# TingweiMeng/PDHG-optimal-control

Measured on AMD Instinct MI355X. Metric: PDHG iterations/sec and achieved HBM GB/s on nt×nx[×ny] grid, 1/2/4/8 MI355X, higher is better.
Workload: dtype f64

## Files before the change

### pdhg-optimal-control_amd/csrc/ctx_impl.hpp

```cpp
#pragma once

#include <hip/hip_runtime.h>

#include <algorithm>
#include <climits>
#include <cmath>
#include <cstring>
#include <map>
#include <memory>
#include <string>
#include <type_traits>
#include <utility>
#include <vector>

#include "kernels_1d.hpp"
#include "kernels_2d.hpp"
#include "kernels_2d_fast.hpp"
#include "kernels_dual_lds.hpp"
#include "kernels_dual_multi.hpp"
#include "kernels_common.hpp"
#include "kernels_xslab.hpp"
#include "kernels_xt_batch.hpp"
#include "kernels_xt_dma.hpp"
#include "kernels_thomas_chunk.hpp"
// ... 608 lines not shown
          default: return fail(PDHG_ERR_UNSUPPORTED, "no batched x kernel for nx=%d", p.nx);
        }
        if (pp.fast_xt_code == 2) switch (p.nx) {
          case 8192: return launch(k_precond_xt_ws_2d<4096, 1, true>, g, dim3(512), lds, p, twx);
          case 4096: return launch(k_precond_xt_ws_2d<4096, 1>, g, dim3(512), lds, p, twx);
          case 2048: return launch(k_precond_xt_ws_2d<2048, 2>, g, dim3(512), lds, p, twx);
          case 1024: return launch(k_precond_xt_ws_2d<1024, 4>, g, dim3(512), lds, p, twx);
          case 512: return launch(k_precond_xt_ws_2d<512, 8>, g, dim3(512), lds, p, twx);
          default: return fail(PDHG_ERR_UNSUPPORTED, "no fast x kernel for nx=%d", p.nx);
        }
        switch (p.nx) {
          case 4096: return launch(k_precond_xt_fast_2d<4096, 1, 512>, g, dim3(512), lds, p, twx);
          case 2048: return launch(k_precond_xt_fast_2d<2048, 2, 512>, g, dim3(512), lds, p, twx);
          case 1024: return launch(k_precond_xt_fast_2d<1024, 4, 512>, g, dim3(512), lds, p, twx);
          case 512: return launch(k_precond_xt_fast_2d<512, 8, 512>, g, dim3(512), lds, p, twx);
          default: return fail(PDHG_ERR_UNSUPPORTED, "no fast x kernel for nx=%d", p.nx);
        }
      }
    } else {
      if (pp.t1_xt64 && one_row) {
        const bool g16 = pp.t1_g16;
        const size_t lds = (size_t)((p.B / 2) * (p.nx + p.nx / 16) + (g16 ? 48 : twlds_size(p.nx))) * sizeof(C);
        switch (p.nx) {
          case 4096:
            if (g16) return launch(k_precond_x_t1_2d<4096, 1, 512, double, true>, g, dim3(512), lds, p, twx);
            return launch(k_precond_x_t1_2d<4096, 1, 512, double>, g, dim3(512), lds, p, twx);
          case 2048:
            if (g16) return launch(k_precond_x_t1_2d<2048, 1, 256, double, true>, g, dim3(256), lds, p, twx);
            return launch(k_precond_x_t1_2d<2048, 1, 256, double>, g, dim3(256), lds, p, twx);
          case 1024: return launch(k_precond_x_t1_2d<1024, 2, 512, double>, g, dim3(512), lds, p, twx);
          case 512: return launch(k_precond_x_t1_2d<512, 4, 512, double>, g, dim3(512), lds, p, twx);
          default: return fail(PDHG_ERR_UNSUPPORTED, "no fp64 one-row x kernel for nx=%d", p.nx);
        }
      }
      if (pp.f64_xt) {
        if (pp.half_real)
          return launch(k_precond_xt_f64_2d<4096, 512, true>, g, dim3(512),
                        (size_t)(Pad<4096>::LINE + TwLds<4096>::SIZE + 4096 + 128) * sizeof(C), p, twx);
        if (p.nx == 1024)
          return launch(k_precond_xt_f64_2d<1024, 256, false, true>, g, dim3(256),
                        (size_t)(Pad<1024>::LINE + TwLds<1024>::SIZE) * sizeof(C), p, twx);
        if (p.nx == 512)
          return launch(k_precond_xt_f64_2d<512, 128, false, true>, g, dim3(128),
                        (size_t)(Pad<512>::LINE + TwLds<512>::SIZE) * sizeof(C), p, twx);
        if (p.nx == 2048) {
          const size_t bpr = (size_t)(Pad<2048>::LINE + TwLds<2048>::SIZE) * sizeof(C);
          switch (pp.xt64_var) {
            case 1: return launch(k_precond_xt_f64_2d<2048, 256, false, false>, g, dim3(256), bpr + 2048 * sizeof(C), p, twx);
            case 2: return launch(k_precond_xt_f64_2d<2048, 256, false, true>, g, dim3(256), bpr, p, twx);
            case 3: return launch(k_precond_xt_f64_2d<2048, 1024, false, true>, g, dim3(1024), bpr, p, twx);
            default: return launch(k_precond_xt_f64_2d<2048, 512, false, true>, g, dim3(512), bpr, p, twx);
          }
        }
        if (pp.xt64_dma) {
          if (p.rspec) return launch(k_precond_xt_f64_2d<4096, 512, false, true, true, true>, g, dim3(512), 0, p, twx);
          return launch(k_precond_xt_f64_2d<4096, 512, false, true, false, true>, g, dim3(512), 0, p, twx);
        }
        if (pp.xt64_bpr) {
          const size_t ldsr = (size_t)(Pad<4096>::LINE + TwLds<4096>::SIZE) * sizeof(C);
          if (p.rspec) return launch(k_precond_xt_f64_2d<4096, 512, false, true, true>, g, dim3(512), ldsr, p, twx);
          return launch(k_precond_xt_f64_2d<4096, 512, false, true>, g, dim3(512), ldsr, p, twx);
        }
        const size_t lds = (size_t)(Pad<4096>::LINE + TwLds<4096>::SIZE + 4096) * sizeof(C);
        if (p.rspec)
          return launch(k_precond_xt_f64_2d<4096, 512, false, false, true>, g, dim3(512), lds, p, twx);
        return launch(k_precond_xt_f64_2d<4096, 512>, g, dim3(512), lds, p, twx);
      }
    }
    return with_xt_fft([&](auto f) {
      return launch(k_precond_xt_2d<R, decltype(f)>, g, dim3(pp.NT2), pp.lds_xt, p, f, twx);
    });
  }

  int launch_update_2d(const KP<R>& p, int& upd_rows) {
    ProfScope ps(this, "update");
    const dim3 gf(pp.g_fast_upd);
    upd_rows = pp.g_fast_upd;
    if constexpr (sizeof(R) == 8) {
      if (pp.res64) {
        if (pb.ny == 2048 && pp.upd_t1 > 0) {
          const size_t lds = pp.lds_res64 + (size_t)48 * sizeof(C);
          if (pp.upd_t1 == 2) return launch(k_invy_update_fast_2d<2048, 4, 256, 2, double, true>, gf, dim3(256), lds, p, twy);
          return launch(k_invy_update_fast_2d<2048, 4, 256, 4, double, true>, gf, dim3(256), lds, p, twy);
        }
        if (pb.ny == 4096) return launch(k_invy_update_fast_2d<4096, 4, 512, 4, double>, gf, dim3(512), pp.lds_upd64, p, twy);
        return launch(k_invy_update_fast_2d<2048, 4, 512, 4, double>, gf, dim3(512), pp.lds_upd64, p, twy);
      }
      if (pp.upd8192)
        return launch(k_invy_update_fast_2d<8192, 2, 512, 2, double>, gf, dim3(512),
                      (size_t)Pad<8192>::LINE * sizeof(C), p, twy);
    }
    if constexpr (kMixed) {
      if (pp.fast_rows)
        return with_fast_rows([&](auto Nc, auto RWc, auto NTc) {
          constexpr int N_ = decltype(Nc)::value, RW_ = decltype(RWc)::value, NT_ = decltype(NTc)::value;
          if constexpr (NT_ == 1024 && RW_ == 8) {
            if (pp.upd_threads == 512)
              return launch(k_invy_update_fast_mixed_2d<N_, RW_, 512, kMixedUpdPF>, gf, dim3(512), pp.lds_fast_tw, p,
                            twy, px);
          }
          return launch(k_invy_update_fast_mixed_2d<N_, RW_, NT_>, gf, dim3(NT_), pp.lds_fast_tw, p, twy, px);
        });
      upd_rows = pp.gx4 * pp.g4;
      return with_line_fft(pp.ply, [&](auto f) {
        using F = decltype(f);
        if (pp.nt_row <= 256)
          return launch(k_invy_update_mixed_2d<F, 256>, dim3(pp.gx4), dim3(pp.nt_row), pp.lds_res, p, f, twy, px);
        return launch(k_invy_update_mixed_2d<F, 1024>, dim3(pp.gx4), dim3(pp.nt_row), pp.lds_res, p, f, twy, px);
      });
    }
    if (pp.fast_rows)
      return with_fast_rows([&](auto Nc, auto RWc, auto NTc) {
        constexpr int N_ = decltype(Nc)::value, RW_ = decltype(RWc)::value, NT_ = decltype(NTc)::value;
        if constexpr (sizeof(R) == 4) {
          if constexpr (NT_ == 1024 && RW_ == 8) {
            if (pp.upd_threads == 512) switch (pp.upd_pf) {
              case 2: return launch(k_invy_update_fast_2d<N_, RW_, 512, 2>, gf, dim3(512), pp.lds_fast_tw, p, twy);
              case 3: return launch(k_invy_update_fast_2d<N_, RW_, 512, 3>, gf, dim3(512), pp.lds_fast_tw, p, twy);
              case 4: return launch(k_invy_update_fast_2d<N_, RW_, 512, 4>, gf, dim3(512), pp.lds_fast_tw, p, twy);
              default: return launch(k_invy_update_fast_2d<N_, RW_, 512, 1>, gf, dim3(512), pp.lds_fast_tw, p, twy);
            }
          }
          return launch(k_invy_update_fast_2d<N_, RW_, NT_>, gf, dim3(NT_), pp.lds_fast_tw, p, twy);
        }
        return (int)PDHG_OK;
      });
    upd_rows = pp.gx4 * pp.g4;
    return with_line_fft(pp.ply, [&](auto f) {
      using F = decltype(f);
      if (pp.nt_row <= 256)
        return launch(k_invy_update_2d<R, F, 256>, dim3(pp.gx4), dim3(pp.nt_row), pp.lds_res, p, f, twy);
      return launch(k_invy_update_2d<R, F, 1024>, dim3(pp.gx4), dim3(pp.nt_row), pp.lds_res, p, f, twy);
    });
  }

  int launch_primal(R tau, int stages = 7, int xt_phase = 0, double* sums_out = nullptr) {
    KP<R> p = kp;
    p.tau = tau;
    p.xt_phase = xt_phase;
    const int T = pb.T;
    int rc;
    if (pb.ndim == 2) {
      if ((stages & 1) && (rc = launch_residual(p, 0, T))) return rc;
      if ((stages & 2) && (rc = launch_precond(p))) return rc;
      if (!(stages & 4)) return PDHG_OK;
      const bool prim_merge = spec && pp.fin_merge && !pp.dual_multi && !sums_out;
      if (prim_merge) p.partials = prim_partials;
      int upd_rows = 0;
      if ((rc = launch_update_2d(p, upd_rows))) return rc;
      if (sums_out)
        return launch(k_reduce_vec, dim3(1), dim3(1024), 0, p.partials, upd_rows, 3, kp.j0 == 0 ? row0_sq : 0.0,
                      sums_out);
      if (prim_merge) {
        prim_merged_rows = upd_rows;
        return PDHG_OK;
      }
      return launch(k_finalize_primal, dim3(1), dim3(1024), 0, p.partials, upd_rows, 1, p.ctrl);
    }
    if constexpr (kMixed) return fail(PDHG_ERR_STATE, "mixed context is 2-D only");
    if (pp.fourstep) return launch_fourstep_1d(p);
    {
      ProfScope ps(this, "residual");
      rc = with_line_fft(pp.plx, [&](auto f) {
        using F = decltype(f);
        return with_egno<2>([&](auto eg) {
          return launch(k_res_fwdx_1d<R, decltype(eg)::value, F>, dim3(pp.gx1), dim3(pp.nt1d), pp.lds_res, p, f, twx);
// ... 1189 lines not shown
```

### pdhg-optimal-control_amd/csrc/kernels_2d_fast.hpp

```cpp
#pragma once
#include <type_traits>
#include "params.hpp"

namespace pdhg {

__device__ __forceinline__ float4 ld4(const float* p) { return *reinterpret_cast<const float4*>(p); }
__device__ __forceinline__ void st4(float* p, float4 v) { *reinterpret_cast<float4*>(p) = v; }
__device__ __forceinline__ float f4(const float4& v, int e) { return e == 0 ? v.x : e == 1 ? v.y : e == 2 ? v.z : v.w; }
__device__ __forceinline__ void f4set(float4& v, int e, float x) {
  if (e == 0) v.x = x; else if (e == 1) v.y = x; else if (e == 2) v.z = x; else v.w = x;
}
__device__ __forceinline__ float4 z4() { return make_float4(0.f, 0.f, 0.f, 0.f); }

struct dbl4 {
  double x, y, z, w;
};
template <typename R> struct V4s { using type = float4; };
template <> struct V4s<double> { using type = dbl4; };
template <typename R> using V4 = typename V4s<R>::type;
__device__ __forceinline__ dbl4 ld4(const double* p) {
  const double2 a = reinterpret_cast<const double2*>(p)[0], b = reinterpret_cast<const double2*>(p)[1];
  return dbl4{a.x, a.y, b.x, b.y};
}
__device__ __forceinline__ void st4(double* p, dbl4 v) {
// ... 643 lines not shown
      }
#pragma unroll
      for (int i = 0; i < BATCH; ++i) {
        const int t = tl + (i0 + i) * NT;
        const int b = t >> lCS4, part = t & (CS4 - 1);
        if (B == 2) {
          C* Al = A + part * Pad<N>::LINE;
          Al[pix(2 * b)] = cmk<C>(v[i].x, v[i].z);
          Al[pix(2 * b + 1)] = cmk<C>(v[i].y, v[i].w);
        } else {
#pragma unroll
          for (int e = 0; e < 4; ++e) {
            const int f = part * 4 + e;
            const int r = f >> lB, c = f & (B - 1);
            Af[((r >> 1) * Pad<N>::LINE + pix(b * B + c)) * 2 + (r & 1)] = f4(v[i], e);
          }
        }
      }
    }
    R* phi = p.phi + (size_t)(j + 1) * plane;
    R* pbar = p.phibar + (size_t)(j + 1) * plane;
    constexpr int NS = GPT * NL;
    V op[NS][2];
    auto ldstep = [&](int s) {
      const size_t idx = (size_t)(x0 + 2 * (s % NL)) * N + 4 * (tid + (s / NL) * NT);
      op[s][0] = ld4(phi + idx);
      op[s][1] = ld4(phi + idx + N);
    };
    ldstep(0);
    lds_sync();
    if (!(p.dbg & 64)) {
      if constexpr (TWL && G16) lds_fft_inplace_tl16<C, N, NL, NT, Pad<N>::LINE>(A, twl, twy);
      else if constexpr (TWL) lds_fft_inplace_tl<C, N, NL, NT, Pad<N>::LINE>(A, twl);
      else lds_fft_inplace<C, N, NL, NT>(A, twy);
    }
#pragma unroll
    for (int s = 1; s < PF && s < NS; ++s) ldstep(s);
#pragma unroll
    for (int gi = 0; gi < GPT; ++gi) {
      const int y = 4 * (tid + gi * NT);
#pragma unroll
      for (int l = 0; l < NL; ++l) {
        const int st = gi * NL + l;
        const V o4[2] = {op[st][0], op[st][1]};
        if (st + PF < NS) ldstep(st + PF);
        const C* Z = A + l * Pad<N>::LINE;
        V u[2];
#pragma unroll
        for (int e = 0; e < 4; ++e) {
          R a, b2;
          hartley_padded<C, R>(Z, N, y + e, a, b2);
          f4set(u[0], e, a);
          f4set(u[1], e, b2);
        }
#pragma unroll
        for (int h = 0; h < 2; ++h) {
          const int xr = x0 + 2 * l + h;
          if (xr < p.xl0 || xr >= p.xl1) continue;
          const size_t idx = (size_t)xr * N + y;
          V nw, pb;
          R fs[3] = {(R)0, (R)0, (R)0};
#pragma unroll
          for (int e = 0; e < 4; ++e) {
            const R o = f4(o4[h], e);
            const R n = o + scale * f4(u[h], e);
            f4set(nw, e, n);
            f4set(pb, e, (R)2 * n - o);
            const R d = n - o;
            fs[0] = fmar(d, d, fs[0]);
            fs[1] = fmar(o, o, fs[1]);
            fs[2] = fmar(n, n, fs[2]);
          }
#pragma unroll
          for (int i = 0; i < 3; ++i) s[i] += (double)fs[i];
          st4(phi + idx, nw);
          st4(pbar + idx, pb);
        }
      }
    }
    lds_sync();
  }
  block_reduce_store<3>(s, p.partials, blockIdx.x);
}
template <int N, int RW, int NT, int PF = 1>
__global__ void __launch_bounds__(NT) k_invy_update_fast_mixed_2d(KP<float> p, const float2* __restrict__ twy,
                                                                  PhiX<float, double> px) {
  invy_update_fast_body<N, RW, NT, PF, float, false, double>(p, px, twy);
}

}

namespace pdhg {

__device__ __forceinline__ float expm1_neg(float x) {
  const float p = x * (1.f + x * (0.5f + x * (1.f / 6 + x * (1.f / 24 + x * (1.f / 120 + x * (1.f / 720 + x * (1.f / 5040)))))));
  return x > -0.25f ? p : __expf(x) - 1.f;
}

__device__ __forceinline__ float2 expm1_neg2(float a, float b) {
  float ea = __expf(a) - 1.f, eb = __expf(b) - 1.f;
  const bool sa = a > -0.25f, sb = b > -0.25f;
  if (__ballot(sa || sb) != 0) {
    auto poly = [](float x) {
      return x * (1.f + x * (0.5f + x * (1.f / 6 + x * (1.f / 24 + x * (1.f / 120 + x * (1.f / 720 + x * (1.f / 5040)))))));
    };
    if (sa) ea = poly(a);
    if (sb) eb = poly(b);
  }
  return make_float2(ea, eb);
}

__device__ __forceinline__ float h_entry(float dd, int j0) {
  if (j0 == 0) return 1.f;
  const float dl = 0.5f * dd;
  const float th = fmaxf(log1pf(dl + sqrtf(dl * (dl + 2.f))), 1e-20f);
  return expm1f(-th) * (1.f + expf(-th * (float)(2 * j0 + 1))) / expm1f(-2.f * th * (float)(j0 + 1));
}
__device__ __forceinline__ double h_entry(double dd, int j0) {
  if (j0 == 0) return 1.0;
  const double dl = 0.5 * dd;
  const double th = fmax(log1p(dl + sqrt(dl * (dl + 2.0))), 1e-300);
  return expm1(-th) * (1.0 + exp(-th * (double)(2 * j0 + 1))) / expm1(-2.0 * th * (double)(j0 + 1));
}

template <int N, int NL, int NT>
__global__ void __launch_bounds__(NT) k_precond_xt_fast_2d(KP<float> p, const float2* __restrict__ twx) {
  using C = float2;
  constexpr int IT = N * NL / NT;
  constexpr int B = 2 * NL;
  constexpr int NI = N * NL;
  constexpr int LINE = Pad<N>::LINE;
  constexpr int lnl = (NL == 1) ? 0 : (NL == 2) ? 1 : (NL == 4) ? 2 : 3;
  if (p.ctrl->done) return;
  extern __shared__ __align__(16) unsigned char smem_raw[];
  C* A = reinterpret_cast<C*>(smem_raw);
  C* sth = A + NL * LINE;
  C* sE = sth + NI;
  C* sbp = sE + NI;
  const int T = p.T, tid = threadIdx.x;
  const int b = blockIdx.x + p.b0;
  constexpr int M = N * B;
  float* wb = p.work + (size_t)b * M;
  const size_t kstride = (size_t)p.nb * M;
  const float ae = p.ae, inv_ae = 1.f / ae;
  C* twl = sbp + NI;
  fill_twlds<C, N>(twl, twx);
  C pf[IT], pf2[IT];
  auto ldrow = [&](C (&dstv)[IT], int kk) {
    const C* sn = reinterpret_cast<const C*>(wb + (size_t)kk * kstride);
#pragma unroll
    for (int i = 0; i < IT; ++i) dstv[i] = sn[tid + i * NT];
  };
#pragma unroll
  for (int i = 0; i < IT; ++i) {
    const int item = tid + i * NT;
    const int kx = item >> lnl, l = item & (NL - 1);
    const float lx = p.lamx[kx];
    const float dd0 = (p.C - lx - p.lamy[b * B + 2 * l]) * inv_ae, dd1 = (p.C - lx - p.lamy[b * B + 2 * l + 1]) * inv_ae;
    sth[item] = make_float2(dd0, dd1);
    sE[item] = make_float2(h_entry(dd0, p.j0), h_entry(dd1, p.j0));
    sbp[item] = make_float2(0.f, 0.f);
  }
  if (p.xt_phase != 2) {
  ldrow(pf, 0);
  ldrow(pf2, min(1, T - 1));
  for (int k = 0; k < T; ++k) {
// ... 643 lines not shown
```

### pdhg-optimal-control_amd/csrc/path_plan.hpp

```cpp
#pragma once

#include <cstdio>
#include <string>

#include "../../include/pdhg.h"
#include "fft_lds.hpp"
#include "kernels_dual_multi.hpp"
#include "kernels_fs16.hpp"
#include "tuning.hpp"

namespace pdhg {

constexpr size_t kLdsBytes = 160 * 1024;
constexpr int kMultiSub = 5;
constexpr int kMixedUpdPF = 4;
constexpr int kFoldRows = 64;

inline FFTPlan make_plan(int n, bool& ok) {
  FFTPlan pl{};
  pl.n = n;
  pl.pow2 = (n > 0) && ((n & (n - 1)) == 0);
  int m = n, np = 0;
  ok = true;
  auto push = [&](int r) {
    if (np >= kMaxPass) { ok = false; return; }
    pl.radix[np++] = r;
  };
  for (int r : {16, 8, 4, 2})
    while (m % r == 0 && m > 1) { push(r); m /= r; }
  while (m % 3 == 0) { push(3); m /= 3; }
  for (int f = 5; m > 1; f += 2)
    while (m % f == 0) { push(f); m /= f; }
  pl.npass = np;
  return pl;
}

struct Decomp {
  bool slab = false;
  int j0 = 0, Tg = 0;
  bool xslab = false;
  int rank = 0, P = 1, nxg = 0, nloc = 0;
  bool mixed = false;
};

struct PathPlan {
  FFTPlan plx{}, ply{};
  int na = 0, n_dead = 0;
  bool mixed = false;
  bool two_sets = false;
  int B = 1, lB = 0, nb = 1, tile_j = 0;
  bool half_real = false;
  int xs_nbs = 0;
  int NT2 = 512;
  int gx1 = 0, gx4 = 0, g4 = 1, gx5 = 0, g5 = 1, g_outer = 1;
  int head_xrun = 4;
  int nt_row = 256;
  int rows_var = 0;
  int res64_nt = 512;
  int half_nt = 3;
  int upd_pf = 4;
  int NTd = 256, gxd = 0, gyd = 0, gzd = 0, jchunk_d = 1;
  int gz_1d = 1, jchunk_1d = 1;
  int nt1d = 256;
  int RWf = 8, NTf = 1024, g_fast_upd = 1;
  size_t partial_rows = 0;
  size_t lds_res = 0, lds_xt = 0, lds_batch_xt = 0, lds_fast_xt = 0, lds_fast = 0, lds_fast_tw = 0, lds_res64 = 0,
         lds_upd64 = 0;
  bool fast_dual = false;
  int dual_rx = 0;
  int dual_ypl = 4;
  int dual_order = 0;
  int dual_one = 0;
  bool dual_multi = false;
  bool dual_head = false;
  bool k1_outer = true;
  bool fold_fin = false;
  bool spec_ok = false;
  bool fin_merge = true;
  bool fuse_res = false;
  bool fast_rows = false;
  bool res64 = false;
  bool ip_rows = false;
  bool upd8192 = false;
  bool tc_spec = false;
  bool to_c4 = false;
  int res_threads = 0, upd_threads = 0;
  int res64_nt2048 = 512;
  int upd_t1 = 0;
  bool t1_xt = true;
  bool fast_xt = false;
  int fast_xt_code = 0;
  bool xt_dma = false, xt_pair = false;
  int xt_rpre = 0;
  bool t1_xt64 = false;
  bool t1_g16 = false;
  bool f64_xt = false;
  int xt64_var = 0;
  bool xt64_bpr = false;
  bool xt64_dma = false;
  bool glb_line = false;
  bool fourstep = false;
  bool fs_wide = true;
  bool fs16 = false;
  int f16_group = 16;
  bool thomas_chunk = false;
  bool report_tile = false;
  int report_wgs = 1024;
};

inline int plan_paths(const pdhg_problem& pb, int S, const Decomp& dc, const Tuning& tn, PathPlan& pl,
                      std::string& err) {
  auto fail = [&err](int code, const char* fmt, auto... args) {
    if constexpr (sizeof...(args) == 0) {
      err = fmt;
    } else {
      char buf[512];
      snprintf(buf, sizeof(buf), fmt, args...);
      err = buf;
    }
    return code;
  };
  pl = PathPlan{};
  if (dc.mixed && (S != 4 || pb.ndim != 2 || dc.slab || dc.xslab))
    return fail(PDHG_ERR_UNSUPPORTED, "mixed precision (12) is implemented for single 2-D contexts only");
  pl.mixed = dc.mixed;
  const int nx = pb.nx, ny = pb.ny, T = pb.T;
  const int nxg = dc.xslab ? dc.nxg : nx;
  const bool is2d = pb.ndim == 2, slab = dc.slab, xslab = dc.xslab;
  const size_t csz = 2 * (size_t)S;
  pl.na = (pb.ndim == 1 || pb.egno == 3) ? 2 : 4;
  pl.n_dead = (pb.ndim == 2 && pb.egno == 3) ? 2 : 0;
  const bool two_sets = pl.two_sets = pb.rho_alp_iters > 1;
  bool ok1 = true, ok2 = true;
  pl.plx = make_plan(nxg, ok1);
  if (is2d) pl.ply = make_plan(ny, ok2);
  if (!ok1 || !ok2) return fail(PDHG_ERR_UNSUPPORTED, "FFT plan too deep for nx=%d ny=%d", nxg, ny);

  if (is2d) {
    const size_t cap = (S == 4) ? 8192 : 4096;
    int B = 16;
    while (B > 2 && (size_t)nxg * B > cap) B >>= 1;
    int nyp = 2;
    while (nyp < ny) nyp <<= 1;
    if (B > nyp) B = nyp;
    const bool xt64_on = tn.xt64.value_or(1) != 0;
    const bool f64_small = S == 8 && pb.bc_x == 0 && (slab ? dc.Tg : T) > 1 && (nxg == 1024 || nxg == 512) &&
                           ny % 2 == 0 && xt64_on;
    if (f64_small) B = 2;
    pl.half_real = nxg == 8192 && pb.bc_x == 0 && (S == 4 || !xslab);
    if (pl.half_real) B = 1;
    pl.f64_xt = S == 8 && pb.bc_x == 0 &&
                (((nxg == 4096 || nxg == 2048) && B == 2) || (nxg == 8192 && pl.half_real) || f64_small) && xt64_on;
    pl.xt64_var = tn.xt64_var;
    {
      const bool ok = pl.f64_xt && nxg == 4096 && B == 2 && !pl.half_real && !slab && !xslab;
      const bool dma = ok && tn.xt64_dma.value_or(1) != 0;
      pl.xt64_bpr = ok && tn.xt64_bpr.value_or(dma ? 1 : 0) != 0;
      pl.xt64_dma = dma && pl.xt64_bpr;
    }
    pl.t1_xt64 = S == 8 && T == 1 && pb.bc_x == 0 && !pl.half_real && !slab && pl.plx.pow2 &&
                 nxg >= 512 && nxg <= 4096 && nxg * (B / 2) == (nxg == 4096 ? 4096 : 2048);
    pl.res64_nt2048 = tn.res64_nt2048.value_or(T == 1 ? 256 : 512);
    pl.upd_t1 = T == 1 ? tn.upd_t1.value_or(2) : 0;
    if (!pl.half_real && !pl.f64_xt && (size_t)nxg * B > cap)
      return fail(PDHG_ERR_UNSUPPORTED, "nx=%d too large for the x-transform slab (max %zu in this precision)", nxg,
                  cap / 2);
// ... 11 lines not shown
    {
      const int wg = (int)std::max<size_t>(1, kLdsBytes / std::max<size_t>(pl.lds_res, 1));
      pl.nt_row = std::min(1024, 256 * std::max(1, 4 / wg));
    }
    pl.NT2 = std::min(512, ((nmodes + 63) / 64) * 64);
    pl.gx1 = ((nx + 1) / 2) * T;
    pl.gx4 = (int)std::min<long long>((long long)pl.gx1, 4096);
    pl.gx5 = (ny + 255) / 256;
    pl.g5 = std::max(1, std::min(T * nx, 8192 / std::max(1, pl.gx5)));
    pl.t1_xt = tn.t1_xt;
    pl.k1_outer = tn.k1_outer;
    pl.fold_fin = tn.fold_fin;
    const bool short_win = T < tn.short_t_xt, short_dual = T < tn.short_t_dual;
    bool ws_xt = false, batch_xt = false, xt_dma_hr = false;
    if (pl.half_real && S == 4) {
      pl.fast_xt = true;
      ws_xt = true;
      xt_dma_hr = tn.xt_dma_hr ? *tn.xt_dma_hr != 0 : T >= 4;
      pl.lds_fast_xt = (size_t)(2 * (4096 + 4096 / 16) + 816 + 4096) * csz;
    } else if (S == 4 && pl.plx.pow2 && nxg * (B / 2) == 4096 && nxg >= 512 && pb.bc_x == 0) {
      pl.fast_xt = true;
      ws_xt = tn.xt_ws ? *tn.xt_ws != 0 : (nxg == 4096) && !short_win;
      batch_xt = tn.xt_batch ? *tn.xt_batch != 0 : (nxg == 4096 || nxg == 2048) && T >= 4;
      pl.xt_rpre = tn.xt_rpre;
      pl.xt_pair = tn.xt_pair;
      pl.xt_dma = nxg == 4096 && tn.xt_dma.value_or(1) != 0;
      pl.lds_batch_xt = (size_t)(4 * (4096 + 4096 / 16) + twlds_size(nxg)) * csz;
      pl.lds_fast_xt = ws_xt ? (size_t)(2 * (4096 + 4096 / 16) + 816) * csz
                             : (size_t)(4096 + 4096 / 16 + 3 * 4096 + 816) * csz;
    }
    pl.fast_xt_code = !pl.fast_xt ? 0 : (pl.half_real && xt_dma_hr) ? 5
                      : (batch_xt && !pl.half_real) ? ((pl.xt_dma && pb.nx == 4096) ? 4 : 3) : ws_xt ? 2 : 1;
    pl.t1_g16 = pl.t1_xt64 && pl.t1_xt && tn.t1_g16 && (nxg == 2048 || nxg == 4096);
    const bool dual64 = S == 8 && ny % 256 == 0 && tn.dual64.value_or(1) != 0;
    int dual_one = 1;
    if ((S == 4 || dual64) && ny % 256 == 0) {
      pl.fast_dual = true;
      pl.dual_rx = (nx % 8 == 0 && !short_dual && !two_sets) ? 8 : 0;
      if (tn.dual_rx) {
        const int v = *tn.dual_rx;
        if (v == 0 || (((S == 4 && (v == 4 || v == 16)) || v == 8) && nx % v == 0)) pl.dual_rx = v;
      }
      if (dc.mixed) pl.dual_rx = 0;
      if (S == 8 && pl.dual_rx == 8 && tn.dual_ypl.value_or(0) == 2) pl.dual_ypl = 2;
      dual_one = tn.dual_one;
      pl.NTd = pl.dual_rx ? pl.dual_rx * 64 : std::min(256, ny / 4);
      pl.gxd = pl.dual_rx ? nx / pl.dual_rx : nx;
      pl.gyd = pl.dual_rx ? ny / (64 * pl.dual_ypl) : (ny / 4 + pl.NTd - 1) / pl.NTd;
      const int nJ0 = std::max(1, std::min(T, (2048 + pl.gxd * pl.gyd - 1) / (pl.gxd * pl.gyd)));
      pl.jchunk_d = (T + nJ0 - 1) / nJ0;
      pl.gzd = (T + pl.jchunk_d - 1) / pl.jchunk_d;
    }
    pl.dual_one = (pl.fast_dual && !pl.dual_rx && pl.jchunk_d == 1) ? dual_one : 0;
    pl.rows_var = tn.rows_var;
    pl.half_nt = tn.half_nt;
    pl.res64_nt = tn.res64_nt;
    pl.upd_pf = tn.upd_pf;
    if (S == 4 && pl.ply.pow2 && ny >= 256 && ny <= 8192) {
      pl.RWf = (ny == 8192) ? 4 : 8;
      pl.NTf = std::min(1024, ny / 4);
      if (pl.rows_var == 1 && (ny == 4096 || ny == 2048)) {
        pl.RWf = 4;
        pl.NTf = ny / 8;
      }
      if (nx % pl.RWf == 0 && (pl.RWf * B) % 4 == 0) {
        pl.fast_rows = true;
        pl.tile_j = ((nx / pl.RWf) % 4 == 0) ? 8 : 1;
        if (tn.tile_j) {
          const int v = *tn.tile_j;
          if (v >= 1 && (v == 1 || (nx / pl.RWf) % 4 == 0)) pl.tile_j = v;
        }
        pl.lds_fast = (size_t)(pl.RWf / 2) * (ny + ny / 16) * csz;
        pl.lds_fast_tw = pl.lds_fast + (ny <= 4096 ? (size_t)twlds_size(ny) * csz : 0);
        pl.g_fast_upd = std::min((nx / pl.RWf) * T, 2048);
      }
    }
    if (S == 8 && pl.ply.pow2 && (ny == 2048 || ny == 4096) && nx % 4 == 0) {
      pl.res64 = tn.res64.value_or(1) != 0;
      if (pl.res64) {
        pl.tile_j = ((nx / 4) % 4 == 0) ? 8 : 1;
        pl.lds_res64 = (size_t)2 * (ny + ny / 16) * csz;
        pl.lds_upd64 = pl.lds_res64 + (size_t)twlds_size(ny) * csz;
        pl.g_fast_upd = std::min((nx / 4) * T, 2048);
      }
    }
    const bool tc_ok = S == 8 && pl.res64 && ny == 4096 && pl.f64_xt && !pl.half_real && nxg == 4096 && B == 2 &&
                       !xslab && T > 1 && !pl.t1_xt64;
    pl.tc_spec = tc_ok && (tn.tc_spec ? *tn.tc_spec != 0 : T >= 100);
    const bool fr_rows = S == 4 ? (pl.fast_rows && (pl.RWf == 8 || (pl.RWf == 4 && ny == 8192)))
                                : ((pl.res64 && (ny == 4096 || ny == 2048)) || (pl.ip_rows && ny == 8192));
    if (pl.fast_dual && pl.dual_rx == 8 && fr_rows && pb.bc_x == 0 && pb.bc_y == 0 && pb.egno != 3 && !two_sets &&
        !xslab) {
      pl.fuse_res = tn.fuse_res ? *tn.fuse_res != 0 : pl.gxd * pl.gyd >= 1024;
      if (pl.fuse_res) {
        if (S == 8) {
          pl.dual_ypl = 2;
          pl.gyd = ny / 128;
        }
        pl.jchunk_d = T;
        pl.gzd = 1;
      }
    }
    const bool band_dflt = pl.fuse_res && pl.gxd * pl.gyd >= 1024 && (ny == 2048 || ny == 4096);
    pl.dual_order = (pl.dual_rx && !slab && !xslab) ? tn.dual_order.value_or(band_dflt ? 1 : 0) : 0;
    pl.to_c4 = pl.fuse_res && pl.half_real && B == 1 && ny == 8192 && !xslab &&
               (S == 8 ? pl.ip_rows : (pl.fast_rows && pl.RWf == 4)) && (nx % (S == 8 ? 64 : 128)) == 0 &&
               tn.c4_to.value_or(1) != 0;
    if (pl.fast_rows) {
      pl.res_threads = (pl.NTf == 1024 && (pl.half_nt & 1) && pl.fuse_res) ? 512 : pl.NTf;
      pl.upd_threads = (pl.NTf == 1024 && pl.RWf == 8 && (pl.half_nt & 2)) ? 512 : pl.NTf;
    }
  } else {
    pl.lds_res = 2 * (size_t)nx * csz;
    pl.gx1 = (T + 1) / 2;
    pl.gx4 = std::min(pl.gx1, 2048);
    if (pl.lds_res > kLdsBytes) {
      pl.glb_line = true;
      pl.lds_res = 0;
      pl.nt1d = 1024;
      pl.fourstep = nx == 65536 && tn.fourstep.value_or(1) != 0;
      pl.fs_wide = tn.fs_wide;
      pl.fs16 = pl.fourstep && tn.fs16.value_or(1) != 0;
      if (S == 8 && !pl.fs16) pl.fourstep = false;
      pl.f16_group = tn.f16_group;
    }
    pl.gx5 = (nx + 255) / 256;
    pl.g5 = std::max(1, std::min(T, 8192 / std::max(1, pl.gx5)));
    pl.thomas_chunk = pb.Ct != 0.0 && T <= 16 * 32 && tn.thomas_chunk.value_or(1) != 0;
    pl.fuse_res = pl.fs16 && pb.bc_x == 0 && !two_sets && pb.egno != 3 && nx % 256 == 0 &&
                  tn.fuse_res1d.value_or(1) != 0;
    pl.gz_1d = std::min(tn.fr1d_chunks, T);
    pl.jchunk_1d = (T + pl.gz_1d - 1) / pl.gz_1d;
    pl.gz_1d = (T + pl.jchunk_1d - 1) / pl.jchunk_1d;
  }
  pl.report_tile = is2d && nx % 8 == 0 && ny % 256 == 0 && pb.bc_y == 0 && (pb.bc_x == 0 || pb.bc_x == 1) && !xslab &&
                   tn.report_tile.value_or(1) != 0;
  pl.report_wgs = tn.report_wgs;
  pl.g_outer = tn.g_outer;
  pl.head_xrun = tn.head_xrun;
  const bool multi_ok = is2d && two_sets && pl.fast_dual && pl.dual_rx == 0 && !slab && !xslab &&
                        pb.rho_alp_iters <= kDualMultiMax;
  pl.dual_multi = multi_ok && (tn.dual_multi ? *tn.dual_multi != 0 : (double)T * nx * ny >= (double)(1 << 25));
  pl.dual_head = multi_ok && !pl.dual_multi && tn.dual_head.value_or(1) != 0;
  pl.spec_ok = pl.dual_head && pl.k1_outer && !pl.fold_fin && tn.spec.value_or(1) != 0;
  pl.fin_merge = tn.fin_merge;
  pl.partial_rows = std::max<size_t>(
      {(size_t)pl.gx4 * pl.g4, (size_t)pl.gx5 * pl.g5, (size_t)pl.g_outer, (size_t)pl.g_fast_upd,
       (size_t)pl.gxd * pl.gyd * (pl.gzd + 1), pl.fourstep ? (size_t)9 * ((T + 1) / 2) : 1, 1,
       (pl.dual_multi || pl.dual_head) ? (size_t)kMultiSub * pl.gxd * pl.gyd * pl.gzd : (size_t)1});
  if (xslab) {
    if (!(is2d && (S == 4 ? pl.fast_rows : pl.res64) && pl.fast_dual && (pb.bc_x == 0 || pb.bc_x == 1) &&
          pb.bc_y == 0))
      return fail(PDHG_ERR_UNSUPPORTED, "x-slab decomposition needs ndim 2, bc (0,0) or (1,0) and a power-of-two ny "
                                        "in [256, 8192] (fp32) or ny = 2048 / 4096 (fp64) (fast row and dual kernels)");
    if (pl.nb % dc.P) return fail(PDHG_ERR_UNSUPPORTED, "%d column blocks do not split over %d ranks", pl.nb, dc.P);
    pl.xs_nbs = pl.nb / dc.P;
  }
  if (slab && !(is2d && (pl.fast_rows || S == 8)))
    return fail(PDHG_ERR_UNSUPPORTED, "t-slab decomposition needs ndim 2 and, in fp32, a power-of-two ny in "
                                      "[256, 8192] (fast row kernels)");
  return PDHG_OK;
}

inline bool plan_key(const PathPlan& pl, const pdhg_problem& pb, int S, const std::string& k, int* value) {
  if (k == "fused_residual") *value = pl.fuse_res ? 1 : 0;
  else if (k == "mixed") *value = pl.mixed ? 1 : 0;
  else if (k == "fast_rows") *value = pl.fast_rows ? 1 : 0;
  else if (k == "res64") *value = pl.res64 ? 1 : 0;
  else if (k == "dual_multi") *value = pl.dual_multi ? 1 : 0;
  else if (k == "dual_head") *value = pl.dual_head ? 1 : 0;
  else if (k == "spec") *value = pl.spec_ok ? 1 : 0;
  else if (k == "dual64") *value = (S == 8 && pl.fast_dual) ? 1 : 0;
  else if (k == "fast_dual") *value = pl.fast_dual ? pl.dual_rx : -1;
  else if (k == "dual_ypl") *value = pl.fast_dual && pl.dual_rx ? pl.dual_ypl : 0;
  else if (k == "res64_nt") *value = pl.res64 ? (pb.ny == 2048 ? pl.res64_nt2048 : 512) : 0;
  else if (k == "upd_t1") *value = (pl.res64 && pb.ny == 2048) ? pl.upd_t1 : 0;
  else if (k == "t1_g16") *value = (pl.t1_g16 && (pb.nx == 2048 || pb.nx == 4096)) ? 1 : 0;
  else if (k == "dual_one") *value = pl.dual_one ? 1 : 0;
  else if (k == "fast_xt") *value = pl.fast_xt_code;
  else if (k == "half_real") *value = pl.half_real ? 1 : 0;
  else if (k == "fourstep") *value = pl.fourstep ? 1 : 0;
  else if (k == "glb_line") *value = pl.glb_line ? 1 : 0;
  else if (k == "ip_rows") *value = pl.ip_rows ? 1 : 0;
  else if (k == "upd8192") *value = pl.upd8192 ? 1 : 0;
  else if (k == "tc_spec") *value = pl.tc_spec ? 1 : 0;
  else if (k == "to_c4") *value = pl.to_c4 ? 1 : 0;
  else if (k == "thomas_chunk") *value = pl.thomas_chunk ? 1 : 0;
  else if (k == "fs_wide") *value = (pl.fourstep && pl.fs_wide && !pl.fs16) ? 1 : 0;
  else if (k == "fs16") *value = pl.fs16 ? 1 : 0;
  else if (k == "rows_rw") *value = pl.fast_rows ? pl.RWf : 0;
  else if (k == "row_threads") *value = pl.nt_row;
  else if (k == "res_threads") *value = pl.res_threads;
  else if (k == "upd_threads") *value = pl.upd_threads;
  else if (k == "f64_xt") *value = pl.f64_xt ? 1 : 0;
  else if (k == "xt64_dma") *value = pl.xt64_dma ? 1 : 0;
  else if (k == "xt64_bpr") *value = pl.xt64_bpr ? 1 : 0;
  else if (k == "t1_xt64") *value = (pl.t1_xt64 && pl.t1_xt) ? 1 : 0;
  else if (k == "report_tile") *value = pl.report_tile ? 1 : 0;
  else if (k == "report_wgs") *value = pl.report_tile ? pl.report_wgs : 0;
  else return false;
  return true;
}

}
```

### pdhg-optimal-control_amd/csrc/tuning.hpp

```cpp
#pragma once

#include <algorithm>
#include <cstdlib>
#include <cstring>
#include <optional>

namespace pdhg {

using EnvInt = std::optional<int>;

inline EnvInt env_int(const char* name) {
  const char* e = getenv(name);
  return e ? EnvInt(atoi(e)) : EnvInt();
}
inline int env_int(const char* name, int dflt) { return env_int(name).value_or(dflt); }
inline bool env_flag(const char* name, bool dflt) { return env_int(name, dflt ? 1 : 0) != 0; }

struct Tuning {
  int alloc_mode = 0;

  EnvInt xt64;
  int xt64_var = 0;
  EnvInt xt64_dma;
  EnvInt xt64_bpr;
  bool t1_xt = true;
  bool t1_g16 = true;
  int short_t_xt = 16;
  EnvInt xt_ws;
  EnvInt xt_batch;
  int xt_rpre = 0;
  bool xt_pair = false;
  EnvInt xt_dma;
  EnvInt xt_dma_hr;

  EnvInt upd_t1;
  EnvInt res64_nt2048;
  EnvInt upd8192;
  int rows_var = 0;
  int half_nt = 3;
  int res64_nt = 512;
  int upd_pf = 4;
  EnvInt tile_j;
  EnvInt res64;
  EnvInt tc_spec;
  EnvInt fuse_res;
  EnvInt c4_to;

  int short_t_dual = 3;
  EnvInt dual64;
  EnvInt dual_rx;
  EnvInt dual_ypl;
  int dual_one = 1;
  bool nbsync = false;
  EnvInt dual_order;
  int dbg = 0;

  EnvInt fourstep;
  bool fs_wide = true;
  EnvInt fs16;
  int f16_group = 16;
  EnvInt fuse_res1d;
  int fr1d_chunks = 8;
  EnvInt thomas_chunk;

  bool k1_outer = true;
  bool fold_fin = false;
  int g_outer = 2048;
  int head_xrun = 4;
  EnvInt dual_multi;
  EnvInt dual_head;
  EnvInt spec;
  bool fin_merge = true;

  EnvInt report_tile;
  int report_wgs = 1024;

  static Tuning from_env() {
    Tuning t;
    if (const char* e = getenv("PDHG_ALLOC")) t.alloc_mode = !strcmp(e, "contig") ? 1 : !strcmp(e, "none") ? -1 : 0;
    t.xt64 = env_int("PDHG_XT64");
    t.xt64_var = env_int("PDHG_XT64_VAR", t.xt64_var);
    t.xt64_dma = env_int("PDHG_XT64_DMA");
    t.xt64_bpr = env_int("PDHG_XT64_BPR");
    t.t1_xt = env_flag("PDHG_T1_XT", t.t1_xt);
    t.t1_g16 = env_flag("PDHG_T1_G16", t.t1_g16);
    t.short_t_xt = env_int("PDHG_SHORT_T_XT", t.short_t_xt);
    t.xt_ws = env_int("PDHG_XT_WS");
    t.xt_batch = env_int("PDHG_XT_BATCH");
    t.xt_rpre = env_int("PDHG_XT_RPRE", t.xt_rpre);
    t.xt_pair = env_flag("PDHG_XT_PAIR", t.xt_pair);
    t.xt_dma = env_int("PDHG_XT_DMA");
    t.xt_dma_hr = env_int("PDHG_XT_DMA_HR");
    t.upd_t1 = env_int("PDHG_UPD_T1");
    if ((t.res64_nt2048 = env_int("PDHG_RES64_NT2048"))) t.res64_nt2048 = *t.res64_nt2048 == 256 ? 256 : 512;
    t.upd8192 = env_int("PDHG_UPD8192");
    t.rows_var = env_int("PDHG_ROWS_VAR", t.rows_var);
    t.half_nt = env_int("PDHG_HALF_NT", t.half_nt);
    t.res64_nt = env_int("PDHG_RES64_NT", t.res64_nt) == 1024 ? 1024 : 512;
    t.upd_pf = env_int("PDHG_UPD_PF", t.upd_pf);
    t.tile_j = env_int("PDHG_TILE_J");
    t.res64 = env_int("PDHG_RES64");
    t.tc_spec = env_int("PDHG_TC_SPEC");
    t.fuse_res = env_int("PDHG_FUSE_RES");
    t.c4_to = env_int("PDHG_C4_TO");
    t.short_t_dual = env_int("PDHG_SHORT_T", t.short_t_dual);
    t.dual64 = env_int("PDHG_DUAL64");
    t.dual_rx = env_int("PDHG_DUAL_RX");
    t.dual_ypl = env_int("PDHG_DUAL_YPL");
    t.dual_one = env_int("PDHG_DUAL_ONE", t.dual_one);
    t.nbsync = env_flag("PDHG_DUAL_NBSYNC", t.nbsync);
    if ((t.dual_order = env_int("PDHG_DUAL_ORDER")) && *t.dual_order != 1 && *t.dual_order != 2 && *t.dual_order != 4)
      t.dual_order = 0;
    t.dbg = env_int("PDHG_DBG", t.dbg);
    t.fourstep = env_int("PDHG_FOURSTEP");
    t.fs_wide = env_flag("PDHG_FS_WIDE", t.fs_wide);
    t.fs16 = env_int("PDHG_FS16");
    t.f16_group = env_int("PDHG_F16_GROUP", t.f16_group);
    t.fuse_res1d = env_int("PDHG_FUSE_RES1D");
    t.fr1d_chunks = std::max(1, std::min(32, env_int("PDHG_FR1D_CHUNKS", t.fr1d_chunks)));
    t.thomas_chunk = env_int("PDHG_THOMAS_CHUNK");
    t.k1_outer = env_flag("PDHG_K1_OUTER", t.k1_outer);
    t.fold_fin = env_flag("PDHG_FOLD_FIN", t.fold_fin);
    t.g_outer = std::max(64, std::min(4096, env_int("PDHG_G_OUTER", t.g_outer)));
    t.head_xrun = std::max(1, env_int("PDHG_HEAD_XRUN", t.head_xrun));
    t.dual_multi = env_int("PDHG_DUAL_MULTI");
    t.dual_head = env_int("PDHG_DUAL_HEAD");
    t.spec = env_int("PDHG_SPEC");
    t.fin_merge = env_flag("PDHG_FIN_MERGE", t.fin_merge);
    t.report_tile = env_int("PDHG_REPORT_TILE");
    t.report_wgs = std::max(1, env_int("PDHG_REPORT_WGS", t.report_wgs));
    return t;
  }
};

struct IterTuning {
  EnvInt graph;
  bool spec_force = false;

  static IterTuning from_env() {
    IterTuning t;
    t.graph = env_int("PDHG_GRAPH");
    t.spec_force = env_flag("PDHG_SPEC_FORCE", t.spec_force);
    return t;
  }
};

struct MultiTuning {
  int parts = 2;
  bool kcopy = false;
  int sync_mask = 0;
  bool one_stream = false;
  bool step_fence = false;
  bool peer_fold = false;

  static MultiTuning from_env() {
    MultiTuning t;
    t.parts = std::max(1, env_int("PDHG_MULTI_PARTS", t.parts));
    t.kcopy = env_flag("PDHG_MULTI_KCOPY", t.kcopy);
    if (const char* e = getenv("PDHG_MULTI_SYNC")) t.sync_mask = (int)strtol(e, nullptr, 0);
    t.one_stream = env_flag("PDHG_MULTI_ONESTREAM", t.one_stream);
    t.step_fence = env_flag("PDHG_MULTI_STEP_FENCE", t.step_fence);
    t.peer_fold = env_flag("PDHG_MULTI_PEER_FOLD", t.peer_fold);
    return t;
  }
};

}
```

Measured before the change: 8.676.

## Add paired-column f64 inverse-y update kernel sharing one coalesced work load

Result: faster. 8.823, median of 6 (+1.7%).

```diff
diff --git a/pdhg-optimal-control_amd/csrc/ctx_impl.hpp b/pdhg-optimal-control_amd/csrc/ctx_impl.hpp
--- a/pdhg-optimal-control_amd/csrc/ctx_impl.hpp
+++ b/pdhg-optimal-control_amd/csrc/ctx_impl.hpp
@@ -714,6 +714,18 @@
           const size_t lds = pp.lds_res64 + (size_t)48 * sizeof(C);
           if (pp.upd_t1 == 2) return launch(k_invy_update_fast_2d<2048, 4, 256, 2, double, true>, gf, dim3(256), lds, p, twy);
           return launch(k_invy_update_fast_2d<2048, 4, 256, 4, double, true>, gf, dim3(256), lds, p, twy);
+        }
+        if (pp.upd64_pair) {
+          auto go = [&](auto PFc) {
+            constexpr int PF_ = decltype(PFc)::value;
+            if (pb.ny == 4096) return launch(k_invy_update_pair_2d<4096, 512, PF_>, gf, dim3(512), pp.lds_upd64, p, twy);
+            return launch(k_invy_update_pair_2d<2048, 512, PF_>, gf, dim3(512), pp.lds_upd64, p, twy);
+          };
+          switch (pp.upd_pair_pf) {
+            case 2: return go(IC<2>{});
+            case 3: return go(IC<3>{});
+            default: return go(IC<4>{});
+          }
         }
         if (pb.ny == 4096) return launch(k_invy_update_fast_2d<4096, 4, 512, 4, double>, gf, dim3(512), pp.lds_upd64, p, twy);
         return launch(k_invy_update_fast_2d<2048, 4, 512, 4, double>, gf, dim3(512), pp.lds_upd64, p, twy);
diff --git a/pdhg-optimal-control_amd/csrc/kernels_2d_fast.hpp b/pdhg-optimal-control_amd/csrc/kernels_2d_fast.hpp
--- a/pdhg-optimal-control_amd/csrc/kernels_2d_fast.hpp
+++ b/pdhg-optimal-control_amd/csrc/kernels_2d_fast.hpp
@@ -749,6 +749,135 @@
   }
   block_reduce_store<3>(s, p.partials, blockIdx.x);
 }
+template <int N, int NT, int PF>
+__global__ void __launch_bounds__(NT) k_invy_update_pair_2d(KP<double> p, const cplx<double>* __restrict__ twy) {
+  using R = double;
+  using C = cplx<R>;
+  using V = V4<R>;
+  constexpr int RW = 4, NL = RW / 2;
+  constexpr int GPT = (N / 4) / NT;
+  if (p.ctrl->done) return;
+  extern __shared__ __align__(16) unsigned char smem_raw[];
+  C* A = reinterpret_cast<C*>(smem_raw);
+  R* Af = reinterpret_cast<R*>(A);
+  C* twl = A + NL * Pad<N>::LINE;
+  fill_twlds<C, N>(twl, twy, 1, TwLds<N>::SIZE);
+  const int nx = p.nx, B = p.B, nb = p.nb;
+  const int npx = nx / (2 * RW);
+  const int npair = npx * p.T;
+  const size_t plane = (size_t)nx * N;
+  const R scale = p.tau * p.inv_n;
+  const int lB = p.lB;
+  const int lCS = lB + 1;
+  const int tid = threadIdx.x;
+  constexpr int NLD = 2 * RW * N / 4 / NT, NH = NLD / 2;
+  static_assert((2 * RW * N / 4) % NT == 0 && NLD % 2 == 0 && NLD <= 16 && NT % 32 == 0, "one batch, halved per task");
+  double s[3] = {0.0, 0.0, 0.0};
+  for (int pr = xcd_remap(blockIdx.x, gridDim.x); pr < npair; pr += gridDim.x) {
+    const int j = pr / npx;
+    int x0 = (pr - j * npx) * (2 * RW);
+    const R* wk = p.work + (size_t)j * nb * nx * B;
+    int tl = tid;
+    asm volatile("" : "+v"(tl));
+    const int hi = (tl >> lB) & 1;
+    V cur[NH], held[NH];
+    {
+      V v[NLD];
+#pragma unroll
+      for (int i = 0; i < NLD; ++i) {
+        const int t = (tl ^ ((i & 1) << lB)) + i * NT;
+        v[i] = ld4(wk + ((size_t)(t >> lCS) * nx + x0) * B + (t & (2 * B - 1)) * 4);
+      }
+#pragma unroll
+      for (int k = 0; k < NH; ++k) {
+        cur[k] = hi ? v[2 * k + 1] : v[2 * k];
+        held[k] = hi ? v[2 * k] : v[2 * k + 1];
+      }
+    }
+    auto put = [&](const V (&w)[NH], int odd) {
+#pragma unroll
+      for (int k = 0; k < NH; ++k) {
+        const int b = (tl >> lCS) + (2 * k + odd) * (NT >> lCS), part = tl & (B - 1);
+        if (B == 2) {
+          C* Al = A + part * Pad<N>::LINE;
+          Al[pix(2 * b)] = cmk<C>(w[k].x, w[k].z);
+          Al[pix(2 * b + 1)] = cmk<C>(w[k].y, w[k].w);
+        } else {
+#pragma unroll
+          for (int e = 0; e < 4; ++e) {
+            const int f = part * 4 + e;
+            const int r = f >> lB, c = f & (B - 1);
+            Af[((r >> 1) * Pad<N>::LINE + pix(b * B + c)) * 2 + (r & 1)] = f4(w[k], e);
+          }
+        }
+      }
+    };
+    R* phi = p.phi + (size_t)(j + 1) * plane;
+    R* pbar = p.phibar + (size_t)(j + 1) * plane;
+#pragma unroll 1
+    for (int half = 0; half < 2; ++half, x0 += RW) {
+      constexpr int NS = GPT * NL;
+      V op[NS][2];
+      auto ldstep = [&](int s) {
+        const size_t idx = (size_t)(x0 + 2 * (s % NL)) * N + 4 * (tid + (s / NL) * NT);
+        op[s][0] = ld4(phi + idx);
+        op[s][1] = ld4(phi + idx + N);
+      };
+      ldstep(0);
+      put(cur, half ? 1 - hi : hi);
+      lds_sync();
+      if (!(p.dbg & 64)) lds_fft_inplace_tl<C, N, NL, NT, Pad<N>::LINE>(A, twl);
+#pragma unroll
+      for (int s = 1; s < PF && s < NS; ++s) ldstep(s);
+#pragma unroll
+      for (int gi = 0; gi < GPT; ++gi) {
+        const int y = 4 * (tid + gi * NT);
+#pragma unroll
+        for (int l = 0; l < NL; ++l) {
+          const int st = gi * NL + l;
+          const V o4[2] = {op[st][0], op[st][1]};
+          if (st + PF < NS) ldstep(st + PF);
+          const C* Z = A + l * Pad<N>::LINE;
+          V u[2];
+#pragma unroll
+          for (int e = 0; e < 4; ++e) {
+            R a, b2;
+            hartley_padded<C, R>(Z, N, y + e, a, b2);
+            f4set(u[0], e, a);
+            f4set(u[1], e, b2);
+          }
+#pragma unroll
+          for (int h = 0; h < 2; ++h) {
+            const int xr = x0 + 2 * l + h;
+            if (xr < p.xl0 || xr >= p.xl1) continue;
+            const size_t idx = (size_t)xr * N + y;
+            V nw, pb;
+            R fs[3] = {(R)0, (R)0, (R)0};
+#pragma unroll
+            for (int e = 0; e < 4; ++e) {
+              const R o = f4(o4[h], e);
+              const R n = o + scale * f4(u[h], e);
+              f4set(nw, e, n);
+              f4set(pb, e, (R)2 * n - o);
+              const R d = n - o;
+              fs[0] = fmar(d, d, fs[0]);
+              fs[1] = fmar(o, o, fs[1]);
+              fs[2] = fmar(n, n, fs[2]);
+            }
+#pragma unroll
+            for (int i = 0; i < 3; ++i) s[i] += (double)fs[i];
+            st4(phi + idx, nw);
+            st4(pbar + idx, pb);
+          }
+        }
+      }
+      lds_sync();
+#pragma unroll
+      for (int k = 0; k < NH; ++k) cur[k] = held[k];
+    }
+  }
+  block_reduce_store<3>(s, p.partials, blockIdx.x);
+}
 template <int N, int RW, int NT, int PF = 1>
 __global__ void __launch_bounds__(NT) k_invy_update_fast_mixed_2d(KP<float> p, const float2* __restrict__ twy,
                                                                   PhiX<float, double> px) {
diff --git a/pdhg-optimal-control_amd/csrc/path_plan.hpp b/pdhg-optimal-control_amd/csrc/path_plan.hpp
--- a/pdhg-optimal-control_amd/csrc/path_plan.hpp
+++ b/pdhg-optimal-control_amd/csrc/path_plan.hpp
@@ -82,6 +82,8 @@
   bool res64 = false;
   bool ip_rows = false;
   bool upd8192 = false;
+  bool upd64_pair = false;
+  int upd_pair_pf = 4;
   bool tc_spec = false;
   bool to_c4 = false;
   int res_threads = 0, upd_threads = 0;
@@ -259,6 +261,12 @@
         pl.lds_res64 = (size_t)2 * (ny + ny / 16) * csz;
         pl.lds_upd64 = pl.lds_res64 + (size_t)twlds_size(ny) * csz;
         pl.g_fast_upd = std::min((nx / 4) * T, 2048);
+        const bool pair_ok = !slab && !xslab && (nx / 4) % 2 == 0 && T >= 1 && B >= 2 && B <= 16 && ny % B == 0 &&
+                             !(ny == 2048 && pl.upd_t1 > 0);
+        pl.upd64_pair = pair_ok && (tn.upd_pair ? *tn.upd_pair != 0 : T >= 100);
+        pl.upd_pair_pf = tn.upd_pair_pf;
+        if (pl.upd64_pair) pl.g_fast_upd = std::min((nx / 8) * T, 2048);
+        if (tn.upd_grid) pl.g_fast_upd = std::min(pl.g_fast_upd, *tn.upd_grid);
       }
     }
     const bool tc_ok = S == 8 && pl.res64 && ny == 4096 && pl.f64_xt && !pl.half_real && nxg == 4096 && B == 2 &&
@@ -360,6 +368,8 @@
   else if (k == "glb_line") *value = pl.glb_line ? 1 : 0;
   else if (k == "ip_rows") *value = pl.ip_rows ? 1 : 0;
   else if (k == "upd8192") *value = pl.upd8192 ? 1 : 0;
+  else if (k == "upd64_pair") *value = pl.upd64_pair ? 1 : 0;
+  else if (k == "upd_grid") *value = pl.g_fast_upd;
   else if (k == "tc_spec") *value = pl.tc_spec ? 1 : 0;
   else if (k == "to_c4") *value = pl.to_c4 ? 1 : 0;
   else if (k == "thomas_chunk") *value = pl.thomas_chunk ? 1 : 0;
diff --git a/pdhg-optimal-control_amd/csrc/tuning.hpp b/pdhg-optimal-control_amd/csrc/tuning.hpp
--- a/pdhg-optimal-control_amd/csrc/tuning.hpp
+++ b/pdhg-optimal-control_amd/csrc/tuning.hpp
@@ -36,6 +36,9 @@
   EnvInt upd_t1;
   EnvInt res64_nt2048;
   EnvInt upd8192;
+  EnvInt upd_pair;
+  int upd_pair_pf = 4;
+  EnvInt upd_grid;
   int rows_var = 0;
   int half_nt = 3;
   int res64_nt = 512;
@@ -94,6 +97,9 @@
     t.upd_t1 = env_int("PDHG_UPD_T1");
     if ((t.res64_nt2048 = env_int("PDHG_RES64_NT2048"))) t.res64_nt2048 = *t.res64_nt2048 == 256 ? 256 : 512;
     t.upd8192 = env_int("PDHG_UPD8192");
+    t.upd_pair = env_int("PDHG_UPD_PAIR");
+    t.upd_pair_pf = std::max(2, std::min(4, env_int("PDHG_UPD_PAIR_PF", t.upd_pair_pf)));
+    if ((t.upd_grid = env_int("PDHG_UPD_GRID"))) t.upd_grid = std::max(1, *t.upd_grid);
     t.rows_var = env_int("PDHG_ROWS_VAR", t.rows_var);
     t.half_nt = env_int("PDHG_HALF_NT", t.half_nt);
     t.res64_nt = env_int("PDHG_RES64_NT", t.res64_nt) == 1024 ? 1024 : 512;
```
